# aurelienpierreeng/ansel

Measured on AMD Instinct MI355X. Metric: MPix/s full export pixelpipe (100 MP raw); % MI355X HBM roofline, higher is better.
Workload: dtype f32

## Files before the change

ansel_amd/csrc/diffuse.hip:

```cpp
#include "hip_common.h"

#include <type_traits>
#include "devmath.h"
#include "ieee_inrange.h"
#include "px_colorspaces.h"

#include <math.h>
#include <cstdlib>

namespace ansel
{
int bspline_launch_decompose(int devid, hipStream_t s, const float4 *in, float4 *hf, float4 *lf, int w, int h, int mult,
                             const unsigned *gate = nullptr);
int bspline_launch_decompose3(int devid, hipStream_t s, const void *in, bool in4, float *lf, int w, int h, int mult, unsigned *alpha_flag);
#ifdef ANSEL_HIP_MEASURING
int bspline_launch_decompose2(int devid, hipStream_t s, const float4 *in, float4 *low1, float4 *low2, int w, int h, int mult);
#endif
}
using namespace ansel;

namespace
{

#define DIFFUSE_MAX_SCALES 10
#define BSPLINE_SIGMA 1.0553651328015339f
#define PDE_KAPPA 0.25f

__device__ __forceinline__ float max_first(const float a, const float b) { return a > b ? a : b; }
__device__ __forceinline__ float max_zero(const float v) { return isfinite(v) ? max_first(v, 0.0f) : 0.0f; }
__device__ __forceinline__ int clampi(const int v, const int lo, const int hi) { return v < lo ? lo : (v > hi ? hi : v); }

__device__ __forceinline__ int walk_row(const int b, const int height, const int mult)
{
  if(height <= mult) return b < height ? b : -1;
  const int per_pass = (height + mult - 1) / mult;
  const int row = (b % per_pass) * mult + b / per_pass;
  return row < height ? row : -1;
}

struct pde_args
{
  int width, height, mult;
  float anisotropy[4];
  int kind[4];
  int same02, same13;
  float variance_threshold, regularization;
  float abcd[4], strength;
  int wskip;
  int post_lab;
  float post_m[3][4];
  int approx_div;
  int off;
  const unsigned *gate;
  int gate_sense;
};

#ifdef ANSEL_HIP_MEASURING
#define PDE_APPROX(a) ((a).approx_div != 0)
#define PDE_OFF(a, bit) (((a).off & (bit)) != 0)
#else
#define PDE_APPROX(a) false
#define PDE_OFF(a, bit) false
#endif
__device__ __forceinline__ float div_1ulp(const float x, const float y)
{
  const float r = __builtin_amdgcn_rcpf(y);
  const float q = x * r;
  return __builtin_fmaf(__builtin_fmaf(-y, q, x), r, q);
}

__device__ __forceinline__ float fast_expf(const float x)
{
  const float t = 1065353216.0f + x * 11401300.0f;
  int k = (t > -2147483648.0f && t < 2147483648.0f) ? (int)t : 0;
  k = k > 0 ? k : 0;
  return __int_as_float(k);
}
// ... 56 lines not shown
    w.k1 = a11;
    w.k2 = -w.k0;
    w.k3 = a00;
    w.k4 = -2.0f * (a00 + a11);
  }
  return w;
}

__device__ __forceinline__ float convolve(const kernel5 w, const float p[9])
{
  float d = 0.0f;
  d = w.k0 * p[0] + d;
  d = w.k1 * p[1] + d;
  d = w.k2 * p[2] + d;
  d = w.k3 * p[3] + d;
  d = w.k4 * p[4] + d;
  d = w.k3 * p[5] + d;
  d = w.k2 * p[6] + d;
  d = w.k1 * p[7] + d;
  d = w.k0 * p[8] + d;
  return d;
}

__device__ __forceinline__ float ratio2(const float h, const float l)
{
  const float safe = max_zero(l - 1e-8f) + 1e-8f;
  const float ratio = h / safe;
  return ratio * ratio;
}
__device__ __forceinline__ float4 ratio2_rgb(const float4 h, const float4 l, const float w_ratio, const bool approx = false)
{
  if(approx)
  {
    const float ax = div_1ulp(h.x, max_zero(l.x - 1e-8f) + 1e-8f), ay = div_1ulp(h.y, max_zero(l.y - 1e-8f) + 1e-8f),
                az = div_1ulp(h.z, max_zero(l.z - 1e-8f) + 1e-8f);
    return make_float4(ax * ax, ay * ay, az * az, w_ratio);
  }
  const float sx = max_zero(l.x - 1e-8f) + 1e-8f, sy = max_zero(l.y - 1e-8f) + 1e-8f, sz = max_zero(l.z - 1e-8f) + 1e-8f;
  const float top = __builtin_fmaxf(__builtin_fmaxf(__builtin_fmaxf(__builtin_fabsf(h.x), __builtin_fabsf(h.y)), __builtin_fabsf(h.z)),
                                    __builtin_fmaxf(__builtin_fmaxf(sx, sy), sz));
  float rx, ry, rz;
  if(__builtin_amdgcn_ballot_w64(!(top <= 0x1p64f)) == 0ull)
  {
    rx = ansel_ieee::div_core(h.x, sx);
    ry = ansel_ieee::div_core(h.y, sy);
    rz = ansel_ieee::div_core(h.z, sz);
  }
  else
  {
    rx = h.x / sx;
    ry = h.y / sy;
    rz = h.z / sz;
  }
  return make_float4(rx * rx, ry * ry, rz * rz, w_ratio);
}

#define PDE_MODE_ISOTROPIC (81 + 162)
#define PDE_MODE_DEBLUR (1 + 9 + 81 + 162)
#define PDE_MODE_ISOPHOTE (1 + 3 + 9 + 27 + 81 + 162)
#define PDE_MODE_GRADIENT (2 + 6 + 18 + 54 + 81 + 162)
#define PDE_MODE_WATERCOLOR (9 + 27)
#define PDE_MODE_CONTRAST (2 + 54)
#define PDE_MODE_INPAINT (27)
#define PDE_MODE_FAST (9)
#define PDE_MODES(X) X(PDE_MODE_ISOTROPIC) X(PDE_MODE_DEBLUR) X(PDE_MODE_ISOPHOTE) X(PDE_MODE_GRADIENT) X(PDE_MODE_WATERCOLOR) \
  X(PDE_MODE_CONTRAST) X(PDE_MODE_INPAINT) X(PDE_MODE_FAST)
template <int MODE> struct pde_mode
{
  static __device__ __forceinline__ int kind(const int i, const pde_args &a)
  {
    if constexpr(MODE < 0) return a.kind[i];
    else return (i == 0 ? MODE : (i == 1 ? MODE / 3 : (i == 2 ? MODE / 9 : MODE / 27))) % 3;
  }
  static __device__ __forceinline__ bool same02(const pde_args &a)
  {
    if constexpr(MODE < 0) return a.same02 != 0;
    else return (MODE / 81) % 2 != 0;
  }
  static __device__ __forceinline__ bool same13(const pde_args &a)
  {
    if constexpr(MODE < 0) return a.same13 != 0;
    else return (MODE / 162) % 2 != 0;
  }
};
inline int pde_mode_of(const pde_args &a)
{
  return a.kind[0] + 3 * a.kind[1] + 9 * a.kind[2] + 27 * a.kind[3] + 81 * (a.same02 ? 1 : 0) + 162 * (a.same13 ? 1 : 0);
}

template <int MODE = -1>
__device__ __forceinline__ float pde_channel(const float H[9], const float L[9], float energy, const pde_args &a)
{
  typedef pde_mode<MODE> M;
  energy = max_zero(a.variance_threshold + energy * a.regularization - 1e-8f) + 1e-8f;
  float cos2g = 0.f, sin2g = 0.f, csg = 0.f, cos2l = 0.f, sin2l = 0.f, csl = 0.f, mg = 0.f, ml = 0.f;
  if(M::kind(0, a) | M::kind(2, a)) mg = direction((L[7] - L[1]) * 0.5f, (L[5] - L[3]) * 0.5f, cos2g, sin2g, csg, PDE_APPROX(a));
  if(M::kind(1, a) | M::kind(3, a)) ml = direction((H[7] - H[1]) * 0.5f, (H[5] - H[3]) * 0.5f, cos2l, sin2l, csl, PDE_APPROX(a));
  const kernel5 w0 = order_kernel(M::kind(0, a), fast_expf(-mg * a.anisotropy[0]), csg, cos2g, sin2g);
  const kernel5 w1 = order_kernel(M::kind(1, a), fast_expf(-ml * a.anisotropy[1]), csl, cos2l, sin2l);
  const kernel5 w2 = M::same02(a) ? w0 : order_kernel(M::kind(2, a), fast_expf(-mg * a.anisotropy[2]), csg, cos2g, sin2g);
  const kernel5 w3 = M::same13(a) ? w1 : order_kernel(M::kind(3, a), fast_expf(-ml * a.anisotropy[3]), csl, cos2l, sin2l);
  const float d0 = convolve(w0, L);
  const float d1 = convolve(w1, L);
  const float d2 = convolve(w2, H);
  const float d3 = convolve(w3, H);
  float update = d0 * a.abcd[0];
  update = d1 * a.abcd[1] + update;
  update = d2 * a.abcd[2] + update;
  update = d3 * a.abcd[3] + update;
  const float acc = H[4] * a.strength + (PDE_APPROX(a) ? div_1ulp(update, energy) : update / energy);
  return max_zero(acc + L[4]);
}

__device__ __forceinline__ bool alpha_is_blank(const float4 H4[9], const float4 L4[9])
{
  unsigned bits = 0;
#pragma unroll
  for(int k = 0; k < 9; k++) bits |= __float_as_uint(H4[k].w) | __float_as_uint(L4[k].w);
  return __builtin_amdgcn_ballot_w64(bits != 0) == 0ull;
}

#define PDE_SHARED_MULT 128
template <bool SHARED>
__global__ __launch_bounds__(256) void diffuse_pde(const float4 *__restrict__ hf, const float4 *__restrict__ lf,
                                                   float4 *__restrict__ out, const pde_args a, const int final_pass,
                                                   const unsigned char *__restrict__ mask)
{
  extern __shared__ float4 r2s[];
// ... 140 lines not shown
  if constexpr(H0_4)
    asm volatile("s_waitcnt lgkmcnt(0)\n\ts_nop 4\n\ts_mov_b32 %0, m0\n\t"
                 "s_mov_b32 m0, %6\n\ts_nop 0\n\tglobal_load_lds_dwordx4 %1, %3\n\t"
                 "s_mov_b32 m0, %7\n\ts_nop 0\n\tglobal_load_lds_dwordx3 %2, %4\n\t"
                 "s_mov_b32 m0, %8\n\ts_nop 0\n\tglobal_load_lds_dwordx3 %2, %5\n\t"
                 "s_mov_b32 m0, %0"
                 : "=&s"(keep)
                 : "v"(voff0), "v"(voff), "s"(p0), "s"(p1), "s"(p2), "s"(d0), "s"(d1), "s"(d2)
                 : "memory");
  else
    asm volatile("s_waitcnt lgkmcnt(0)\n\ts_nop 4\n\ts_mov_b32 %0, m0\n\t"
                 "s_mov_b32 m0, %5\n\ts_nop 0\n\tglobal_load_lds_dwordx3 %1, %2\n\t"
                 "s_mov_b32 m0, %6\n\ts_nop 0\n\tglobal_load_lds_dwordx3 %1, %3\n\t"
                 "s_mov_b32 m0, %7\n\ts_nop 0\n\tglobal_load_lds_dwordx3 %1, %4\n\t"
                 "s_mov_b32 m0, %0"
                 : "=&s"(keep)
                 : "v"(voff), "s"(p0), "s"(p1), "s"(p2), "s"(d0), "s"(d1), "s"(d2)
                 : "memory");
}
struct pde_px3
{
  float x, y, z;
};
template <bool HSUB, int MODE, bool DMA, int L3>
__device__ __forceinline__ void pde_strip_body(const float4 *__restrict__ hf, const float4 *__restrict__ hsub,
                                               const float4 *__restrict__ lf, float4 *__restrict__ out, const pde_args &a,
                                               const int final_pass, const unsigned char *__restrict__ mask, const int strip,
                                               const int strips_per_class)
{
  static_assert(L3 == 0 || (HSUB && DMA), "three-float planes: the low-pass chain's LDS-DMA form only");
  if(a.gate && ((*a.gate != 0u) == (a.gate_sense == 1))) return;
  extern __shared__ float4 r2s[];
  pde_px3 *const r2s3 = reinterpret_cast<pde_px3 *>(r2s);
  const int mult = a.mult;
  const int cls = blockIdx.y / strips_per_class, k0s = (blockIdx.y - cls * strips_per_class) * strip;
  const int n_cls = (a.height - cls + mult - 1) / mult;
  if(k0s >= n_cls) return;
  const int nrows = (strip < n_cls - k0s) ? strip : n_cls - k0s;
  const int r_first = cls + k0s * mult;
  const int tx = threadIdx.x, tw = 256 + 2 * mult;
  const int col = (int)blockIdx.x * 256 + tx;
  const bool live = col < a.width;
  const int cols[3] = { clampi(col - mult, 0, a.width - 1), clampi(col, 0, a.width - 1), clampi(col + mult, 0, a.width - 1) };
#define PDE_ROW(v) ((size_t)clampi(r_first + ((v) - 1) * mult, 0, a.height - 1) * a.width)
  float4 Hw[3][3], Lw[3][3];
  constexpr int NPL = HSUB ? 3 : 2;
  const int lane = tx & 63, zw = 64 + 2 * mult;
  float4 *const zone = r2s + PDE_RING * tw + (tx >> 6) * NPL * zw;
  float4 *const zone3 = reinterpret_cast<float4 *>(reinterpret_cast<char *>(r2s) + (size_t)PDE_RING * tw * 12) + (tx >> 6) * 3 * zw;
  using lds_f4_ptr = __attribute__((address_space(3))) float4 *;
  const unsigned zone_lds = !DMA ? 0u : (unsigned)__builtin_amdgcn_readfirstlane((int)(unsigned)(__UINTPTR_TYPE__)(lds_f4_ptr)(
                                           L3 ? zone3 : zone));
  const unsigned off_main = (unsigned)cols[0] * 16u, off_halo = (unsigned)clampi(col - mult + 64, 0, a.width - 1) * 16u;
  auto dma_row = [&](const int v) {
// ... 9 lines not shown
        pde_dma_planes3<L3 == 2>(b0, b1, b2, L3 == 2 ? off_halo : h3, h3, zone_lds + 1024u, zone_lds + p0 + 1024u, zone_lds + p1 + 1024u);
      return;
    }
    const unsigned pl = (unsigned)zw * 16u;
    pde_dma_planes<NPL>(hf + y, hsub + y, lf + y, off_main, zone_lds, zone_lds + pl, zone_lds + (NPL - 1) * pl);
    if(lane < 2 * mult)
      pde_dma_planes<NPL>(hf + y, hsub + y, lf + y, off_halo, zone_lds + 1024u, zone_lds + pl + 1024u, zone_lds + (NPL - 1) * pl + 1024u);
  };
  struct
  {
    float4 o;
    size_t idx;
    bool have;
  } pending;
  pending.have = false;
  auto store = [&](const size_t i, const float4 o) {
    if(final_pass) nt_store(out + i, o);
    else if constexpr(L3 != 0)
    {
      float *const p3 = (float *)out + 3 * i;
      p3[0] = o.x;
      p3[1] = o.y;
      p3[2] = o.z;
    }
    else out[i] = o;
  };
  auto fetch_row = [&](const int v, auto slot_tag) {
    constexpr int SL = decltype(slot_tag)::value;
    const size_t y = PDE_ROW(v);
    float4 c[3], low[3];
    if constexpr(DMA)
    {
      asm volatile("s_waitcnt vmcnt(0)" : : : "memory");
      if constexpr(L3 != 0)
      {
#pragma unroll
        for(int jj = 0; jj < 3; jj++)
        {
          const int x = lane + jj * mult;
          const float4 v0 = zone3[x], v1 = zone3[zw + x], v2 = zone3[2 * zw + x];
          c[jj] = make_float4(v0.x, v0.y, v0.z, 0.0f);
          low[jj] = make_float4(v1.x, v1.y, v1.z, 0.0f);
          Lw[SL][jj] = make_float4(v2.x, v2.y, v2.z, 0.0f);
        }
      }
      else
// ... 18 lines not shown
    {
#pragma unroll
      for(int jj = 0; jj < 3; jj++)
      {
        c[jj] = hf[y + cols[jj]];
        if(HSUB) low[jj] = hsub[y + cols[jj]];
        Lw[SL][jj] = lf[y + cols[jj]];
      }
    }
    __builtin_amdgcn_sched_barrier(0);
#pragma unroll
    for(int jj = 0; jj < 3; jj++)
      Hw[SL][jj] = HSUB ? make_float4(c[jj].x - low[jj].x, c[jj].y - low[jj].y, c[jj].z - low[jj].z, c[jj].w - low[jj].w) : c[jj];
    float4 *const ring = r2s + (v % PDE_RING) * tw;
    auto ratios = [&](const float4 h, const float4 l) {
      const bool blank = a.wskip && __builtin_amdgcn_ballot_w64((__float_as_uint(h.w) | __float_as_uint(l.w)) != 0) == 0ull;
      return ratio2_rgb(h, l, blank ? 0.0f : ratio2(h.w, l.w), PDE_APPROX(a));
    };
    if(PDE_OFF(a, 4)) return;
    if constexpr(L3 != 0)
    {
      pde_px3 *const ring3 = r2s3 + (v % PDE_RING) * tw;
      auto put = [&](const int x, const float4 h, const float4 l) {
        const float4 r = ratio2_rgb(h, l, 0.0f, PDE_APPROX(a));
        ring3[x] = { r.x, r.y, r.z };
      };
      put(tx + mult, Hw[SL][1], Lw[SL][1]);
      if(tx < mult) put(tx, Hw[SL][0], Lw[SL][0]);
      if(tx >= 256 - mult) put(tx + 2 * mult, Hw[SL][2], Lw[SL][2]);
      return;
    }
    ring[tx + mult] = ratios(Hw[SL][1], Lw[SL][1]);
    if(tx < mult) ring[tx] = ratios(Hw[SL][0], Lw[SL][0]);
    if(tx >= 256 - mult) ring[tx + 2 * mult] = ratios(Hw[SL][2], Lw[SL][2]);
  };
  auto row_step = [&](auto t_tag, const int kk) {
    constexpr int T = decltype(t_tag)::value, S0 = T, S1 = (T + 1) % 3, S2 = (T + 2) % 3;
    constexpr bool WIDE_READS = MODE >= 0 && !(((MODE % 3) | ((MODE / 9) % 3)) && (((MODE / 3) % 3) | ((MODE / 27) % 3)));
    fetch_row(kk + 2, std::integral_constant<int, S2>());
    if constexpr(DMA)
    {
      if(pending.have)
      {
        store(pending.idx, pending.o);
        pending.have = false;
      }
      if(kk + 1 < nrows) dma_row(kk + 3);
// ... 38 lines not shown
      {
        const float4 r = ring[jj * mult];
        energy.x += r.x;
        energy.y += r.y;
        energy.z += r.z;
        if(!(blank && a.wskip)) energy.w += r.w;
      }
      if(!WIDE_READS || ii >= 1) asm volatile("" : "+v"(energy.x), "+v"(energy.y), "+v"(energy.z), "+v"(energy.w) : : "memory");
    }
    const size_t idx = (size_t)row * a.width + col;
    float4 o;
    if(L3 == 0 && mask && !mask[idx])
    {
      const float4 h = H4[4], l = L4[4];
      o = make_float4(max_zero(h.x + l.x), max_zero(h.y + l.y), max_zero(h.z + l.z), max_zero(h.w + l.w));
    }
    else if(PDE_OFF(a, 16))
      o = make_float4(H4[4].x + energy.x, L4[4].y + energy.y, H4[0].z + energy.z, L4[8].w);
    else
    {
      float H[9], L[9];
#pragma unroll
      for(int k = 0; k < 9; k++) { H[k] = H4[k].x; L[k] = L4[k].x; }
      o.x = pde_channel<MODE>(H, L, energy.x, a);
#pragma unroll
      for(int k = 0; k < 9; k++) { H[k] = H4[k].y; L[k] = L4[k].y; }
      o.y = pde_channel<MODE>(H, L, energy.y, a);
#pragma unroll
      for(int k = 0; k < 9; k++) { H[k] = H4[k].z; L[k] = L4[k].z; }
      o.z = pde_channel<MODE>(H, L, energy.z, a);
      if(blank)
        o.w = 0.0f;
      else
      {
#pragma unroll
        for(int k = 0; k < 9; k++) { H[k] = H4[k].w; L[k] = L4[k].w; }
        o.w = pde_channel<MODE>(H, L, energy.w, a);
      }
    }
    if(a.post_lab) o = px_rgb_to_lab(o, a.post_m);
    pending.o = o;
    pending.idx = idx;
    pending.have = true;
  };
  if constexpr(DMA) dma_row(0);
  fetch_row(0, std::integral_constant<int, 0>());
  if constexpr(DMA) dma_row(1);
  fetch_row(1, std::integral_constant<int, 1>());
  if constexpr(DMA) dma_row(2);
  for(int kk = 0; kk < nrows; kk += 3)
  {
    row_step(std::integral_constant<int, 0>(), kk);
    if(kk + 1 < nrows) row_step(std::integral_constant<int, 1>(), kk + 1);
    if(kk + 2 < nrows) row_step(std::integral_constant<int, 2>(), kk + 2);
  }
  if constexpr(DMA) asm volatile("s_waitcnt vmcnt(0)" : : : "memory");
  if(pending.have) store(pending.idx, pending.o);
#undef PDE_ROW
}

template <bool HSUB, int MODE, bool DMA = false>
__global__ __launch_bounds__(256, 3) void diffuse_pde_strip(const float4 *__restrict__ hf, const float4 *__restrict__ hsub,
                                                         const float4 *__restrict__ lf,
                                                         float4 *__restrict__ out, const pde_args a, const int final_pass,
                                                         const unsigned char *__restrict__ mask, const int strip,
                                                         const int strips_per_class)
{
  pde_strip_body<HSUB, MODE, DMA, 0>(hf, hsub, lf, out, a, final_pass, mask, strip, strips_per_class);
}
template <int MODE, bool H0_4>
__global__ __launch_bounds__(256, 3) void diffuse_pde_strip3(const float4 *__restrict__ hf, const float4 *__restrict__ hsub,
                                                          const float4 *__restrict__ lf, float4 *__restrict__ out, const pde_args a,
                                                          const int final_pass, const int strip, const int strips_per_class)
{
  pde_strip_body<true, MODE, true, H0_4 ? 2 : 1>(hf, hsub, lf, out, a, final_pass, nullptr, strip, strips_per_class);
}

__device__ __forceinline__ uint32_t splitmix32(const uint64_t seed)
{
  uint64_t result = (seed ^ (seed >> 33)) * 0x62a9d9ed799705f5ull;
  result = (result ^ (result >> 28)) * 0xcb24d0a5c88c35b3ull;
  return (uint32_t)(result >> 32);
}

__device__ __forceinline__ float xoshiro128plus(uint32_t state[4])
{
  const uint32_t result = state[0] + state[3];
  const uint32_t t = state[1] << 9;
  state[2] ^= state[0];
  state[3] ^= state[1];
  state[1] ^= state[2];
  state[0] ^= state[3];
  state[2] ^= t;
  state[3] = (state[3] << 11) | (state[3] >> 21);
  return (float)(result >> 8) * 0x1.0p-24f;
}

__device__ __forceinline__ float gaussian_noise(const float mu, const float sigma, const bool flip, uint32_t state[4])
// ... 73 lines not shown
int diffuse_halo_rows(const dt_hip_piece_t *piece, const dt_hip_diffuse_data_t *d)
{
  if(!(d->iscale > 0.0f) || !(piece->roi_in.scale > 0.0)) return -1;
  const int scales = scales_of(piece, d);
  const int it_req = (int)ceilf((float)d->iterations);
  const int iterations = it_req > 1 ? it_req : 1;
  return iterations * 3 * ((1 << scales) - 1);
}
}

extern "C" {

int dt_hip_iop_diffuse_process(int devid, const dt_hip_piece_t *piece, const dt_hip_diffuse_data_t *d,
                               dt_hip_mem_t dev_in, dt_hip_mem_t dev_out)
{
  return diffuse_process_rows(devid, piece, d, 0, dev_in, dev_out);
}

}

namespace ansel
{
static void *g_diffuse_probe = nullptr;

static int diffuse_run(int devid, const dt_hip_piece_t *piece, const dt_hip_diffuse_data_t *d, int first_row, dt_hip_mem_t dev_in,
                       dt_hip_mem_t dev_out, const dt_hip_lab_data_t *post_lab);
int diffuse_process_rows(int devid, const dt_hip_piece_t *piece, const dt_hip_diffuse_data_t *d, int first_row,
                         dt_hip_mem_t dev_in, dt_hip_mem_t dev_out)
{
  return diffuse_run(devid, piece, d, first_row, dev_in, dev_out, nullptr);
}
int diffuse_process_post_lab(int devid, const dt_hip_piece_t *piece, const dt_hip_diffuse_data_t *d, dt_hip_mem_t dev_in,
                             dt_hip_mem_t dev_out, const dt_hip_lab_data_t *lab)
{
  if(!lab || measuring_env("ANSEL_HIP_PDE_PER_ROW")) return DT_HIP_INVALID_ARG;
  return diffuse_run(devid, piece, d, 0, dev_in, dev_out, lab);
}
static int diffuse_run(int devid, const dt_hip_piece_t *piece, const dt_hip_diffuse_data_t *d, int first_row, dt_hip_mem_t dev_in,
                       dt_hip_mem_t dev_out, const dt_hip_lab_data_t *post_lab)
{
  if(!valid_device(devid) || !piece || !d || !dev_in || !dev_out) return DT_HIP_INVALID_ARG;
  if(piece->channels != 4)
  {
    set_last_error("diffuse: needs a 4-channel float input");
    return DT_HIP_INVALID_ARG;
  }
// ... 29 lines not shown
    const char *const approx_env = measuring_env("ANSEL_HIP_PDE_APPROX_DIV");
    a.approx_div = approx_env && atoi(approx_env) != 0;
    const char *const off_env = measuring_env("ANSEL_HIP_PDE_OFF");
    a.off = off_env ? atoi(off_env) : 0;
  }
  const float user_aniso[4] = { d->anisotropy_first, d->anisotropy_second, d->anisotropy_third, d->anisotropy_fourth };
  for(int k = 0; k < 4; k++)
  {
    a.anisotropy[k] = sqf(user_aniso[k]);
    a.kind[k] = user_aniso[k] == 0.0f ? 0 : (user_aniso[k] > 0.0f ? 1 : 2);
  }
  a.same02 = a.kind[0] == a.kind[2] && a.anisotropy[0] == a.anisotropy[2];
  a.same13 = a.kind[1] == a.kind[3] && a.anisotropy[1] == a.anisotropy[3];
  const float regularization = powf(10.0f, d->regularization) - 1.0f;
  a.variance_threshold = powf(10.0f, d->variance_threshold);
  const float speed[4] = { d->first, d->second, d->third, d->fourth };

  hipStream_t st = stream_of(devid);
  const float4 *src = (const float4 *)dev_in;
  const int mode0 = pde_mode_of(a);
  const bool three = err == DT_HIP_SUCCESS && lf_chain && !no_dma && !(d->threshold > 0.0f) && (1 << (scales - 1)) <= PDE_DMA_MAX_MULT &&
                     !(iterations == 1 && dev_in == dev_out) && !measuring_env("ANSEL_HIP_PDE_GENERIC") &&
                     (mode0 == PDE_MODE_DEBLUR || mode0 == PDE_MODE_ISOTROPIC);
  unsigned *alpha_flag = nullptr;
  if(three)
  {
    alpha_flag = (unsigned *)dt_hip_alloc_device_buffer(devid, sizeof(unsigned));
    if(!alpha_flag) err = DT_HIP_SYSMEM_ALLOCATION;
    else if(hipMemsetAsync(alpha_flag, 0, sizeof(unsigned), st) != hipSuccess) err = DT_HIP_DEFAULT_ERROR;
  }
  unsigned char *mask = nullptr;
  float4 *inpainted = nullptr;
  if(err == DT_HIP_SUCCESS && d->threshold > 0.0f)
  {
    const size_t np = (size_t)w * h;
    mask = (unsigned char *)dt_hip_alloc_device_buffer(devid, np);
    inpainted = tmp[1] ? tmp[1] : (tmp[1] = (float4 *)dt_hip_alloc_device_buffer(devid, plane));
    if(!mask || !inpainted) err = DT_HIP_SYSMEM_ALLOCATION;
    else
    {
      launch_scope ls(devid, "diffuse_inpaint");
      diffuse_inpaint<<<pixel_grid(np), 256, 0, st>>>(src, inpainted, mask, d->threshold, np, (size_t)w, (size_t)first_row * w);
      err = check_launch("diffuse_inpaint");
      src = inpainted;
    }
  }
  for(int seq = three ? 0 : 1; seq < 2 && err == DT_HIP_SUCCESS; seq++)
  {
  const bool p3 = seq == 0;
  a.gate = alpha_flag;
  a.gate_sense = p3 ? 1 : 2;
  if(three) src = (const float4 *)dev_in;
// ... 5 lines not shown
    const bool chain = lf_chain && (const float4 *)dst != src;
    if(!chain && !lf[1])
    {
      lf[1] = (float4 *)dt_hip_alloc_device_buffer(devid, plane);
      if(!lf[1])
      {
        err = DT_HIP_SYSMEM_ALLOCATION;
        break;
      }
    }
    for(int s = 0; s < scales && err == DT_HIP_SUCCESS; s++)
    {
#ifdef ANSEL_HIP_MEASURING
      static const bool pairs = measuring_env("ANSEL_HIP_BSPLINE_PAIRS") != nullptr;
      if(chain && pairs && s + 1 < scales && (s == 0 || s == 2))
      {
        err = bspline_launch_decompose2(devid, st, level, hf[s], hf[s + 1], w, h, 1 << s);
        s++;
        level = residual = hf[s];
        continue;
      }
#endif
      float4 *low = chain ? hf[s] : lf[s % 2];
      if(p3) err = bspline_launch_decompose3(devid, st, level, it == 0 && s == 0, (float *)low, w, h, 1 << s, alpha_flag);
      else err = bspline_launch_decompose(devid, st, level, chain ? nullptr : hf[s], low, w, h, 1 << s, alpha_flag);
      level = low;
      residual = low;
    }
    float4 *pp[2] = { residual == lf[1] ? lf[0] : lf[1], residual };
    const float4 *cur = residual;
    int count = 0;
    for(int s = scales - 1; s >= 0 && err == DT_HIP_SUCCESS; s--, count++)
    {
      const float real_radius = sigma_at_step(BSPLINE_SIGMA, (unsigned)s) * zoom;
      a.regularization = regularization / 9.0f * sqf(real_radius);
      const float norm = expf(-sqf(real_radius - (float)d->radius_center) / sqf((float)d->radius));
      for(int k = 0; k < 4; k++) a.abcd[k] = speed[k] * PDE_KAPPA * norm;
      a.strength = d->sharpness * norm + 1.0f;
      a.mult = 1 << s;
      a.post_lab = 0;
      if(post_lab && s == 0 && it == iterations - 1)
      {
        a.post_lab = 1;
        memcpy(a.post_m, post_lab->matrix, sizeof(a.post_m));
      }
      float4 *to = (s == 0) ? dst : (chain ? (count % 2 == 0 ? lf[0] : hf[s + 1]) : pp[count % 2]);
      const int rows = (h <= a.mult) ? h : ((h + a.mult - 1) / a.mult) * a.mult;
// ... 11 lines not shown
          if(strip_env) strip = atoi(strip_env);
#endif
          while(strip > 4 && (size_t)gx * classes * ((per_class + strip - 1) / strip) < 2048) strip /= 2;
          const int spc = (per_class + strip - 1) / strip;
          size_t ring = (size_t)PDE_RING * (256 + 2 * a.mult) * sizeof(float4);
#ifdef ANSEL_HIP_MEASURING
          static const char *const pad_env = measuring_env("ANSEL_HIP_PDE_LDS_PAD");
          if(pad_env) ring += (size_t)atoi(pad_env);
#endif
          static const bool generic = measuring_env("ANSEL_HIP_PDE_GENERIC") != nullptr;
          const int mode = generic ? -1 : pde_mode_of(a);
          const dim3 sgrid(gx, classes * spc);
          const float4 *const h0 = chain ? (s == 0 ? src : hf[s - 1]) : hf[s], *const h1 = chain ? hf[s] : nullptr;
#define PDE_LAUNCH(HS, MD) diffuse_pde_strip<HS, MD><<<sgrid, 256, ring, st>>>(h0, h1, cur, to, a, s == 0, mask, strip, spc)
          const bool dma = chain && a.mult <= PDE_DMA_MAX_MULT && !no_dma;
          const size_t ring_dma = ring + (size_t)4 * 3 * (64 + 2 * a.mult) * sizeof(float4);
#define PDE_LAUNCH_DMA(MD) diffuse_pde_strip<true, MD, true><<<sgrid, 256, ring_dma, st>>>(h0, h1, cur, to, a, s == 0, mask, strip, spc)
          bool launched = false;
          if(p3)
          {
            const bool h0_4 = it == 0 && s == 0;
            const size_t lds3 = (size_t)PDE_RING * (256 + 2 * a.mult) * 12 + (size_t)4 * 3 * (64 + 2 * a.mult) * 16;
            const int last = s == 0 && it == iterations - 1;
#define PDE_LAUNCH3(MD, H4) diffuse_pde_strip3<MD, H4><<<sgrid, 256, lds3, st>>>(h0, h1, cur, to, a, last, strip, spc)
            if(mode == PDE_MODE_DEBLUR)
            {
              if(h0_4) PDE_LAUNCH3(PDE_MODE_DEBLUR, true);
              else PDE_LAUNCH3(PDE_MODE_DEBLUR, false);
            }
            else
            {
              if(h0_4) PDE_LAUNCH3(PDE_MODE_ISOTROPIC, true);
              else PDE_LAUNCH3(PDE_MODE_ISOTROPIC, false);
            }
#undef PDE_LAUNCH3
            launched = true;
          }
#define PDE_CASE(MD)                     \
  if(!launched && mode == (MD))          \
  {                                      \
    if(dma) PDE_LAUNCH_DMA(MD);          \
    else if(chain) PDE_LAUNCH(true, MD); \
    else PDE_LAUNCH(false, MD);          \
    launched = true;                     \
  }
          PDE_MODES(PDE_CASE)
#undef PDE_CASE
// ... 5 lines not shown
          }
#undef PDE_LAUNCH_DMA
#undef PDE_LAUNCH
        }
        else if(a.mult <= PDE_SHARED_MULT)
          diffuse_pde<true><<<grid, 256, (size_t)3 * (256 + 2 * a.mult) * sizeof(float4), st>>>(hf[s], cur, to, a, s == 0, mask);
        else
          diffuse_pde<false><<<grid, 256, 0, st>>>(hf[s], cur, to, a, s == 0, mask);
      }
      err = check_launch("diffuse_pde");
      cur = to;
    }
    src = dst;
  }
  }
  for(int s = 0; s < scales; s++)
    if(hf[s]) dt_hip_release_mem_object(hf[s]);
  for(int k = 0; k < 2; k++)
  {
    if(lf[k]) dt_hip_release_mem_object(lf[k]);
    if(tmp[k]) dt_hip_release_mem_object(tmp[k]);
  }
  if(mask) dt_hip_release_mem_object(mask);
  if(alpha_flag)
  {
    if(g_diffuse_probe && err == DT_HIP_SUCCESS && hipMemcpyAsync(g_diffuse_probe, alpha_flag, sizeof(unsigned), hipMemcpyDeviceToDevice, st) != hipSuccess)
      err = DT_HIP_DEFAULT_ERROR;
    dt_hip_release_mem_object(alpha_flag);
  }
  else if(g_diffuse_probe && err == DT_HIP_SUCCESS && hipMemsetAsync(g_diffuse_probe, 0xff, sizeof(unsigned), st) != hipSuccess)
    err = DT_HIP_DEFAULT_ERROR;
  return err;
}

}

extern "C" {

int dt_hip_test_diffuse_probe(void *sink)
{
  ansel::g_diffuse_probe = sink;
  return DT_HIP_SUCCESS;
}

void dt_hip_iop_diffuse_tiling(const dt_hip_piece_t *piece, const dt_hip_diffuse_data_t *d, dt_hip_tiling_t *tiling)
{
  const int scales = scales_of(piece, d);
  tiling->factor = 6.0625f + scales;
  tiling->factor_cl = 6.0625f + scales;
  tiling->maxbuf = 1.0f;
  tiling->maxbuf_cl = 1.0f;
  tiling->overhead = 0;
  tiling->overlap = 1 << scales;
  tiling->xalign = 1;
  tiling->yalign = 1;
}

}
```

ansel_amd/csrc/diffuse_bspline.hip:

```cpp
#include "hip_common.h"

#include <cstdlib>

using namespace ansel;

namespace
{

__device__ __forceinline__ float max_first(const float a, const float b) { return a > b ? a : b; }
__device__ __forceinline__ int clampi(const int v, const int lo, const int hi) { return v < lo ? lo : (v > hi ? hi : v); }

__device__ __forceinline__ float tap5(const float a, const float b, const float c, const float d, const float e)
{
  const float s = 0.0625f * a + 0.25f * b + 0.375f * c + 0.25f * d + 0.0625f * e;
  return max_first(0.0f, s);
}
__device__ __forceinline__ float4 tap5(const float4 a, const float4 b, const float4 c, const float4 d, const float4 e)
{
  return make_float4(tap5(a.x, b.x, c.x, d.x, e.x), tap5(a.y, b.y, c.y, d.y, e.y), tap5(a.z, b.z, c.z, d.z, e.z),
                     tap5(a.w, b.w, c.w, d.w, e.w));
}

__device__ __forceinline__ int walk_row(const int b, const int height, const int mult)
{
// ... 152 lines not shown
    c = d;
    d = e;
    e = n1;
    a2 = b2;
    b2 = c2;
    c2 = d2;
    d2 = e2;
    e2 = n2;
  }
#undef BS_ROW
}

struct bs_px3
{
  float x, y, z;
};
__device__ __forceinline__ bs_px3 tap5(const bs_px3 a, const bs_px3 b, const bs_px3 c, const bs_px3 d, const bs_px3 e)
{
  return { tap5(a.x, b.x, c.x, d.x, e.x), tap5(a.y, b.y, c.y, d.y, e.y), tap5(a.z, b.z, c.z, d.z, e.z) };
}
template <int R, int T, bool IN4>
__global__ __launch_bounds__(256) void bspline_decompose_strip3(const void *__restrict__ in_v, bs_px3 *__restrict__ lf,
                                                                const int width, const int height, const int strip,
                                                                const int strips_per_class, unsigned *__restrict__ alpha_flag)
{
  static_assert(R * T == 256, "a workgroup's columns: one span of 256");
  constexpr int mult = R;
  if(!IN4 && *alpha_flag != 0u) return;
  __shared__ bs_px3 vert[2][(T + 4) * R + 2];
  const float4 *const in4 = static_cast<const float4 *>(in_v);
  const bs_px3 *const in3 = static_cast<const bs_px3 *>(in_v);
  unsigned alpha_bits = 0;
  auto at = [&](const size_t i) -> bs_px3 {
    if constexpr(IN4)
    {
      const float4 v = in4[i];
      alpha_bits |= __float_as_uint(v.w);
      return { v.x, v.y, v.z };
    }
    else
      return in3[i];
  };
  const int cls = blockIdx.y / strips_per_class, k0s = (blockIdx.y - cls * strips_per_class) * strip;
  const int n_cls = (height - cls + mult - 1) / mult;
  if(k0s >= n_cls) return;
  const int nrows = (strip < n_cls - k0s) ? strip : n_cls - k0s;
  const int r_first = cls + k0s * mult;
  const int k0 = (int)blockIdx.x * T;
  const int tid = threadIdx.x;
  const int r = tid % R, k = tid / R;
  const int col = r + (k0 + k) * mult;
  const bool own = col < width;
  int col2 = -1, slot2 = 0;
  if(tid < 4 * R)
  {
    const int hr = tid % R, hs = tid / R;
    const int hk = hs < 2 ? hs - 2 : T + hs - 2;
    const int hcol = hr + (k0 + hk) * mult;
    if(hcol >= 0 && hcol < width)
    {
// ... 31 lines not shown
    d2 = at(BS_ROW(1) + col2);
    e2 = at(BS_ROW(2) + col2);
  }
  for(int kk = 0; kk < nrows; kk++)
  {
    const int row = r_first + kk * mult;
    const bool more = kk + 1 < nrows;
    bs_px3 n1 = z, n2 = z;
    if(more && own) n1 = at(BS_ROW(kk + 3) + col);
    if(more && second) n2 = at(BS_ROW(kk + 3) + col2);
    bs_px3 *const V = vert[kk & 1];
    if(own) V[(k + 2) * R + r] = tap5(a, b, c, d, e);
    if(second) V[slot2] = tap5(a2, b2, c2, d2, e2);
    __syncthreads();
    if(own)
    {
      bs_px3 t[5];
#pragma unroll
      for(int s = -2; s <= 2; s++)
      {
        const int cc = col + s * mult;
        t[s + 2] = cc < 0 ? V[(T + 4) * R] : (cc > width - 1 ? V[(T + 4) * R + 1] : V[(k + s + 2) * R + r]);
      }
      lf[(size_t)row * width + col] = tap5(t[0], t[1], t[2], t[3], t[4]);
    }
    a = b;
    b = c;
    c = d;
    d = e;
    e = n1;
    a2 = b2;
    b2 = c2;
    c2 = d2;
    d2 = e2;
    e2 = n2;
  }
#undef BS_ROW
  if(IN4 && __builtin_amdgcn_ballot_w64(alpha_bits != 0u) != 0ull && (tid & 63) == 0) atomicOr(alpha_flag, 1u);
}

#ifdef ANSEL_HIP_MEASURING
__device__ __forceinline__ float4 bs_row_taps(const float4 *__restrict__ V, const int col, const int step, const int origin,
                                              const int width)
{
  float4 t[5];
#pragma unroll
  for(int j = 0; j < 5; j++) t[j] = V[clampi(col + (j - 2) * step, 0, width - 1) - origin];
  return tap5(t[0], t[1], t[2], t[3], t[4]);
}

template <int M, int AHEAD>
__global__ __launch_bounds__(320) void bspline_decompose2_strip(const float4 *__restrict__ in, float4 *__restrict__ low1,
                                                                float4 *__restrict__ low2, const int width, const int height,
                                                                const int strip, const int strips_per_class)
{
  constexpr int M2 = 2 * M, WA = 256 + 12 * M, WB = 256 + 8 * M;
  static_assert(WA <= 320, "a lane a column");
  __shared__ float4 VA[2][WA], VC[2][WB];
  const int c0 = (int)blockIdx.x * 256;
  const int cls = blockIdx.y / strips_per_class, k0s = (blockIdx.y - cls * strips_per_class) * strip;
  const int n_cls = (height - cls + M2 - 1) / M2;
// ... 112 lines not shown
  static const char *const ahead_env = measuring_env("ANSEL_HIP_BSPLINE_AHEAD");
  const int ahead = ahead_env ? atoi(ahead_env) : 1;
#define BS_PAIR(MM) \
  switch(ahead) \
  { \
    case 2: bspline_decompose2_strip<MM, 2><<<grid, 320, 0, s>>>(in, low1, low2, w, h, strip, spc); break; \
    case 4: bspline_decompose2_strip<MM, 4><<<grid, 320, 0, s>>>(in, low1, low2, w, h, strip, spc); break; \
    case 3: bspline_decompose2_strip<MM, 3><<<grid, 320, 0, s>>>(in, low1, low2, w, h, strip, spc); break; \
    default: bspline_decompose2_strip<MM, 1><<<grid, 320, 0, s>>>(in, low1, low2, w, h, strip, spc); break; \
  }
  if(mult == 1)
  {
    BS_PAIR(1);
  }
  else
  {
    BS_PAIR(4);
  }
#undef BS_PAIR
  return check_launch("diffuse_decompose");
}
#endif

int bspline_launch_decompose3(int devid, hipStream_t s, const void *in, bool in4, float *lf, int w, int h, int mult, unsigned *alpha_flag)
{
  (void)devid;
  if(mult != 1 && mult != 2 && mult != 4 && mult != 8 && mult != 16) return DT_HIP_INVALID_ARG;
  if(in4 && mult != 1) return DT_HIP_INVALID_ARG;
  const int classes = h < mult ? h : mult, per_class = (h + mult - 1) / mult;
  const int gx = (w + 255) / 256;
  int strip = 32;
  while(strip > 4 && (size_t)gx * classes * ((per_class + strip - 1) / strip) < 2048) strip /= 2;
  const int spc = (per_class + strip - 1) / strip;
  const dim3 grid(gx, classes * spc);
  launch_scope ls(devid, "diffuse_decompose");
  bs_px3 *const out = reinterpret_cast<bs_px3 *>(lf);
  if(in4) bspline_decompose_strip3<1, 256, true><<<grid, 256, 0, s>>>(in, out, w, h, strip, spc, alpha_flag);
  else if(mult == 1) bspline_decompose_strip3<1, 256, false><<<grid, 256, 0, s>>>(in, out, w, h, strip, spc, alpha_flag);
  else if(mult == 2) bspline_decompose_strip3<2, 128, false><<<grid, 256, 0, s>>>(in, out, w, h, strip, spc, alpha_flag);
  else if(mult == 4) bspline_decompose_strip3<4, 64, false><<<grid, 256, 0, s>>>(in, out, w, h, strip, spc, alpha_flag);
  else if(mult == 8) bspline_decompose_strip3<8, 32, false><<<grid, 256, 0, s>>>(in, out, w, h, strip, spc, alpha_flag);
  else bspline_decompose_strip3<16, 16, false><<<grid, 256, 0, s>>>(in, out, w, h, strip, spc, alpha_flag);
  return check_launch("diffuse_decompose");
}

int bspline_launch_decompose(int devid, hipStream_t s, const float4 *in, float4 *hf, float4 *lf, int w, int h, int mult,
                             const unsigned *gate)
{
  const int steps = (w + mult - 1) / mult;
  launch_scope ls(devid, "diffuse_decompose");
#ifdef ANSEL_HIP_MEASURING
  static const bool per_row = getenv("ANSEL_HIP_BSPLINE_PER_ROW") != nullptr;
  if(per_row)
  {
    const int rows = (h <= mult) ? h : ((h + mult - 1) / mult) * mult;
    if(mult == 1)
      bspline_decompose<1, 256><<<dim3(xcd_pad((steps + 255) / 256), rows), 256, 0, s>>>(in, hf, lf, w, h, mult, 1, (steps + 255) / 256);
    else if(mult == 2)
      bspline_decompose<2, 128><<<dim3(xcd_pad((steps + 127) / 128), rows), 256, 0, s>>>(in, hf, lf, w, h, mult, 1, (steps + 127) / 128);
    else if(mult == 4)
      bspline_decompose<4, 64><<<dim3(xcd_pad((steps + 63) / 64), rows), 256, 0, s>>>(in, hf, lf, w, h, mult, 1, (steps + 63) / 64);
    else
    {
      const int groups = mult / 8;
      bspline_decompose<8, 32><<<dim3(xcd_pad(((steps + 31) / 32) * groups), rows), 256, 0, s>>>(in, hf, lf, w, h, mult, groups,
// ... 19 lines not shown
```

ansel_amd/csrc/ieee_inrange.h:

```cpp
#pragma once

namespace ansel_ieee
{

__device__ __forceinline__ float div_core(const float a, const float b)
{
  float r = __builtin_amdgcn_rcpf(b);
  const float e = __builtin_fmaf(-b, r, 1.0f);
  r = __builtin_fmaf(e, r, r);
  float q = a * r;
  const float e2 = __builtin_fmaf(-b, q, a);
  q = __builtin_fmaf(e2, r, q);
  const float e3 = __builtin_fmaf(-b, q, a);
  return __builtin_fmaf(e3, r, q);
}

__device__ __forceinline__ float rcp_core(const float b)
{
  float r = __builtin_amdgcn_rcpf(b);
  const float e = __builtin_fmaf(-b, r, 1.0f);
  r = __builtin_fmaf(e, r, r);
  const float e2 = __builtin_fmaf(-b, r, 1.0f);
  const float q = __builtin_fmaf(e2, r, r);
  const float e3 = __builtin_fmaf(-b, q, 1.0f);
// ... 10 lines not shown
  const float q = n * y1;
  const float q1 = __builtin_fmaf(__builtin_fmaf(-d, q, n), y1, q);
  const float q2 = __builtin_fmaf(__builtin_fmaf(-d, q1, n), y1, q1);
  return __builtin_amdgcn_div_fixupf(q2, d, n);
}

__device__ __forceinline__ float sqrt_core(const float x)
{
  const float s = __builtin_amdgcn_sqrtf(x);
  const float down = __uint_as_float(__float_as_uint(s) - 1u), up = __uint_as_float(__float_as_uint(s) + 1u);
  const float r_down = __builtin_fmaf(-down, s, x);
  float t = (0.0f >= r_down) ? down : s;
  const float r_up = __builtin_fmaf(-up, s, x);
  t = (0.0f < r_up) ? up : t;
  return t;
}

__device__ __forceinline__ bool zero_or_above_2m96(const float x)
{
  const unsigned u = __float_as_uint(x);
  return u == 0u || (u - 0x0f800000u) <= (0x7f7fffffu - 0x0f800000u);
}

}
```

Measured before the change: 1625.

## Add range-gated fused PDE kernel with simplified ratio division and isotropic Laplacian

Introduces a fused variant of the three-float PDE strip kernel that uses a fixed isotropic Laplacian stencil and an unconditional refined division for the ratio term. Its correctness rests on a value-range premise. The B-spline decomposition and the fused kernel both check for out-of-range values and set a device flag. Both the fused and the original kernel are launched each time, gated on that flag so only one does real work. This trims the per-pixel ALU cost of the PDE step in exchange for range checks, an extra launch that exits early, and an atomic flag.

```diff
diff --git a/ansel_amd/csrc/diffuse.hip b/ansel_amd/csrc/diffuse.hip
--- a/ansel_amd/csrc/diffuse.hip
+++ b/ansel_amd/csrc/diffuse.hip
@@ -12,7 +12,8 @@
 {
 int bspline_launch_decompose(int devid, hipStream_t s, const float4 *in, float4 *hf, float4 *lf, int w, int h, int mult,
                              const unsigned *gate = nullptr);
-int bspline_launch_decompose3(int devid, hipStream_t s, const void *in, bool in4, float *lf, int w, int h, int mult, unsigned *alpha_flag);
+int bspline_launch_decompose3(int devid, hipStream_t s, const void *in, bool in4, float *lf, int w, int h, int mult, unsigned *alpha_flag,
+                              unsigned *range_flag);
 #ifdef ANSEL_HIP_MEASURING
 int bspline_launch_decompose2(int devid, hipStream_t s, const float4 *in, float4 *low1, float4 *low2, int w, int h, int mult);
 #endif
@@ -53,6 +54,8 @@
   int off;
   const unsigned *gate;
   int gate_sense;
+  unsigned *range;
+  int range_sense;
 };
 
 #ifdef ANSEL_HIP_MEASURING
@@ -155,6 +158,20 @@
   return d;
 }
 
+__device__ __forceinline__ float convolve_iso_fused(const float p[9])
+{
+  float d = __builtin_fmaf(0.25f, p[0], 0.0f);
+  d = __builtin_fmaf(0.5f, p[1], d);
+  d = __builtin_fmaf(0.25f, p[2], d);
+  d = __builtin_fmaf(0.5f, p[3], d);
+  d = -3.0f * p[4] + d;
+  d = __builtin_fmaf(0.5f, p[5], d);
+  d = __builtin_fmaf(0.25f, p[6], d);
+  d = __builtin_fmaf(0.5f, p[7], d);
+  d = __builtin_fmaf(0.25f, p[8], d);
+  return d;
+}
+
 __device__ __forceinline__ float ratio2(const float h, const float l)
 {
   const float safe = max_zero(l - 1e-8f) + 1e-8f;
@@ -186,6 +203,16 @@
     rz = h.z / sz;
   }
   return make_float4(rx * rx, ry * ry, rz * rz, w_ratio);
+}
+
+#ifndef ANSEL_PDE_FUSED_KEEPS_RATIO_TEST
+#define ANSEL_PDE_FUSED_KEEPS_RATIO_TEST 0
+#endif
+__device__ __forceinline__ float4 ratio2_rgb_r(const float4 h, const float4 l)
+{
+  const float sx = max_first(l.x - 1e-8f, 0.0f) + 1e-8f, sy = max_first(l.y - 1e-8f, 0.0f) + 1e-8f, sz = max_first(l.z - 1e-8f, 0.0f) + 1e-8f;
+  const float rx = ansel_ieee::div_core(h.x, sx), ry = ansel_ieee::div_core(h.y, sy), rz = ansel_ieee::div_core(h.z, sz);
+  return make_float4(rx * rx, ry * ry, rz * rz, 0.0f);
 }
 
 #define PDE_MODE_ISOTROPIC (81 + 162)
@@ -221,7 +248,7 @@
   return a.kind[0] + 3 * a.kind[1] + 9 * a.kind[2] + 27 * a.kind[3] + 81 * (a.same02 ? 1 : 0) + 162 * (a.same13 ? 1 : 0);
 }
 
-template <int MODE = -1>
+template <int MODE = -1, bool FUSED = false>
 __device__ __forceinline__ float pde_channel(const float H[9], const float L[9], float energy, const pde_args &a)
 {
   typedef pde_mode<MODE> M;
@@ -233,10 +260,14 @@
   const kernel5 w1 = order_kernel(M::kind(1, a), fast_expf(-ml * a.anisotropy[1]), csl, cos2l, sin2l);
   const kernel5 w2 = M::same02(a) ? w0 : order_kernel(M::kind(2, a), fast_expf(-mg * a.anisotropy[2]), csg, cos2g, sin2g);
   const kernel5 w3 = M::same13(a) ? w1 : order_kernel(M::kind(3, a), fast_expf(-ml * a.anisotropy[3]), csl, cos2l, sin2l);
-  const float d0 = convolve(w0, L);
-  const float d1 = convolve(w1, L);
-  const float d2 = convolve(w2, H);
-  const float d3 = convolve(w3, H);
+  static_assert(!FUSED || MODE >= 0, "the fused Laplacians: kinds spelled at compile time only");
+  constexpr bool F0 = FUSED && (MODE % 3) == 0, F1 = FUSED && ((MODE / 3) % 3) == 0;
+  constexpr bool F2 = (FUSED && (MODE / 81) % 2) ? F0 : (FUSED && ((MODE / 9) % 3) == 0);
+  constexpr bool F3 = (FUSED && (MODE / 162) % 2) ? F1 : (FUSED && ((MODE / 27) % 3) == 0);
+  const float d0 = F0 ? convolve_iso_fused(L) : convolve(w0, L);
+  const float d1 = F1 ? convolve_iso_fused(L) : convolve(w1, L);
+  const float d2 = F2 ? convolve_iso_fused(H) : convolve(w2, H);
+  const float d3 = F3 ? convolve_iso_fused(H) : convolve(w3, H);
   float update = d0 * a.abcd[0];
   update = d1 * a.abcd[1] + update;
   update = d2 * a.abcd[2] + update;
@@ -423,14 +454,17 @@
 {
   float x, y, z;
 };
-template <bool HSUB, int MODE, bool DMA, int L3>
+template <bool HSUB, int MODE, bool DMA, int L3, bool FUSED = false>
 __device__ __forceinline__ void pde_strip_body(const float4 *__restrict__ hf, const float4 *__restrict__ hsub,
                                                const float4 *__restrict__ lf, float4 *__restrict__ out, const pde_args &a,
                                                const int final_pass, const unsigned char *__restrict__ mask, const int strip,
                                                const int strips_per_class)
 {
   static_assert(L3 == 0 || (HSUB && DMA), "three-float planes: the low-pass chain's LDS-DMA form only");
+  static_assert(!FUSED || L3 != 0, "premise R is established for the three-float planes only");
   if(a.gate && ((*a.gate != 0u) == (a.gate_sense == 1))) return;
+  if(L3 != 0 && a.range && ((*a.range != 0u) == (a.range_sense == 1))) return;
+  unsigned long long outside = 0ull;
   extern __shared__ float4 r2s[];
   pde_px3 *const r2s3 = reinterpret_cast<pde_px3 *>(r2s);
   const int mult = a.mult;
@@ -486,6 +520,7 @@
       p3[0] = o.x;
       p3[1] = o.y;
       p3[2] = o.z;
+      if constexpr(FUSED) outside |= __builtin_amdgcn_ballot_w64(ansel_ieee::outside_r3<true>(o.x, o.y, o.z));
     }
     else out[i] = o;
   };
@@ -550,7 +585,7 @@
     {
       pde_px3 *const ring3 = r2s3 + (v % PDE_RING) * tw;
       auto put = [&](const int x, const float4 h, const float4 l) {
-        const float4 r = ratio2_rgb(h, l, 0.0f, PDE_APPROX(a));
+        const float4 r = (FUSED && !ANSEL_PDE_FUSED_KEEPS_RATIO_TEST) ? ratio2_rgb_r(h, l) : ratio2_rgb(h, l, 0.0f, PDE_APPROX(a));
         ring3[x] = { r.x, r.y, r.z };
       };
       put(tx + mult, Hw[SL][1], Lw[SL][1]);
@@ -635,20 +670,20 @@
       float H[9], L[9];
 #pragma unroll
       for(int k = 0; k < 9; k++) { H[k] = H4[k].x; L[k] = L4[k].x; }
-      o.x = pde_channel<MODE>(H, L, energy.x, a);
+      o.x = pde_channel<MODE, FUSED>(H, L, energy.x, a);
 #pragma unroll
       for(int k = 0; k < 9; k++) { H[k] = H4[k].y; L[k] = L4[k].y; }
-      o.y = pde_channel<MODE>(H, L, energy.y, a);
+      o.y = pde_channel<MODE, FUSED>(H, L, energy.y, a);
 #pragma unroll
       for(int k = 0; k < 9; k++) { H[k] = H4[k].z; L[k] = L4[k].z; }
-      o.z = pde_channel<MODE>(H, L, energy.z, a);
+      o.z = pde_channel<MODE, FUSED>(H, L, energy.z, a);
       if(blank)
         o.w = 0.0f;
       else
       {
 #pragma unroll
         for(int k = 0; k < 9; k++) { H[k] = H4[k].w; L[k] = L4[k].w; }
-        o.w = pde_channel<MODE>(H, L, energy.w, a);
+        o.w = pde_channel<MODE, FUSED>(H, L, energy.w, a);
       }
     }
     if(a.post_lab) o = px_rgb_to_lab(o, a.post_m);
@@ -669,6 +704,8 @@
   }
   if constexpr(DMA) asm volatile("s_waitcnt vmcnt(0)" : : : "memory");
   if(pending.have) store(pending.idx, pending.o);
+  if constexpr(FUSED)
+    if(outside != 0ull && lane == 0) atomicOr(a.range, 1u);
 #undef PDE_ROW
 }
 
@@ -687,6 +724,13 @@
                                                           const int final_pass, const int strip, const int strips_per_class)
 {
   pde_strip_body<true, MODE, true, H0_4 ? 2 : 1>(hf, hsub, lf, out, a, final_pass, nullptr, strip, strips_per_class);
+}
+template <int MODE, bool H0_4>
+__global__ __launch_bounds__(256, 3) void diffuse_pde_fused3(const float4 *__restrict__ hf, const float4 *__restrict__ hsub,
+                                                          const float4 *__restrict__ lf, float4 *__restrict__ out, const pde_args a,
+                                                          const int final_pass, const int strip, const int strips_per_class)
+{
+  pde_strip_body<true, MODE, true, H0_4 ? 2 : 1, true>(hf, hsub, lf, out, a, final_pass, nullptr, strip, strips_per_class);
 }
 
 __device__ __forceinline__ uint32_t splitmix32(const uint64_t seed)
@@ -806,6 +850,7 @@
 namespace ansel
 {
 static void *g_diffuse_probe = nullptr;
+static void *g_diffuse_range_probe = nullptr;
 
 static int diffuse_run(int devid, const dt_hip_piece_t *piece, const dt_hip_diffuse_data_t *d, int first_row, dt_hip_mem_t dev_in,
                        dt_hip_mem_t dev_out, const dt_hip_lab_data_t *post_lab);
@@ -881,12 +926,14 @@
   const bool three = err == DT_HIP_SUCCESS && lf_chain && !no_dma && !(d->threshold > 0.0f) && (1 << (scales - 1)) <= PDE_DMA_MAX_MULT &&
                      !(iterations == 1 && dev_in == dev_out) && !measuring_env("ANSEL_HIP_PDE_GENERIC") &&
                      (mode0 == PDE_MODE_DEBLUR || mode0 == PDE_MODE_ISOTROPIC);
-  unsigned *alpha_flag = nullptr;
+  unsigned *alpha_flag = nullptr, *range_flag = nullptr;
   if(three)
   {
     alpha_flag = (unsigned *)dt_hip_alloc_device_buffer(devid, sizeof(unsigned));
-    if(!alpha_flag) err = DT_HIP_SYSMEM_ALLOCATION;
-    else if(hipMemsetAsync(alpha_flag, 0, sizeof(unsigned), st) != hipSuccess) err = DT_HIP_DEFAULT_ERROR;
+    range_flag = (unsigned *)dt_hip_alloc_device_buffer(devid, sizeof(unsigned));
+    if(!alpha_flag || !range_flag) err = DT_HIP_SYSMEM_ALLOCATION;
+    else if(hipMemsetAsync(alpha_flag, 0, sizeof(unsigned), st) != hipSuccess || hipMemsetAsync(range_flag, 0, sizeof(unsigned), st) != hipSuccess)
+      err = DT_HIP_DEFAULT_ERROR;
   }
   unsigned char *mask = nullptr;
   float4 *inpainted = nullptr;
@@ -938,7 +985,7 @@
       }
 #endif
       float4 *low = chain ? hf[s] : lf[s % 2];
-      if(p3) err = bspline_launch_decompose3(devid, st, level, it == 0 && s == 0, (float *)low, w, h, 1 << s, alpha_flag);
+      if(p3) err = bspline_launch_decompose3(devid, st, level, it == 0 && s == 0, (float *)low, w, h, 1 << s, alpha_flag, range_flag);
       else err = bspline_launch_decompose(devid, st, level, chain ? nullptr : hf[s], low, w, h, 1 << s, alpha_flag);
       level = low;
       residual = low;
@@ -996,7 +1043,16 @@
             const bool h0_4 = it == 0 && s == 0;
             const size_t lds3 = (size_t)PDE_RING * (256 + 2 * a.mult) * 12 + (size_t)4 * 3 * (64 + 2 * a.mult) * 16;
             const int last = s == 0 && it == iterations - 1;
-#define PDE_LAUNCH3(MD, H4) diffuse_pde_strip3<MD, H4><<<sgrid, 256, lds3, st>>>(h0, h1, cur, to, a, last, strip, spc)
+#define PDE_LAUNCH3(MD, H4)                                                                      \
+  do                                                                                             \
+  {                                                                                              \
+    a.range = range_flag;                                                                        \
+    a.range_sense = 1;                                                                           \
+    diffuse_pde_fused3<MD, H4><<<sgrid, 256, lds3, st>>>(h0, h1, cur, to, a, last, strip, spc);  \
+    a.range_sense = 2;                                                                           \
+    diffuse_pde_strip3<MD, H4><<<sgrid, 256, lds3, st>>>(h0, h1, cur, to, a, last, strip, spc);  \
+    a.range = nullptr;                                                                           \
+  } while(0)
             if(mode == PDE_MODE_DEBLUR)
             {
               if(h0_4) PDE_LAUNCH3(PDE_MODE_DEBLUR, true);
@@ -1048,6 +1104,15 @@
     if(tmp[k]) dt_hip_release_mem_object(tmp[k]);
   }
   if(mask) dt_hip_release_mem_object(mask);
+  if(range_flag)
+  {
+    if(g_diffuse_range_probe && err == DT_HIP_SUCCESS
+       && hipMemcpyAsync(g_diffuse_range_probe, range_flag, sizeof(unsigned), hipMemcpyDeviceToDevice, st) != hipSuccess)
+      err = DT_HIP_DEFAULT_ERROR;
+    dt_hip_release_mem_object(range_flag);
+  }
+  else if(g_diffuse_range_probe && err == DT_HIP_SUCCESS && hipMemsetAsync(g_diffuse_range_probe, 0xff, sizeof(unsigned), st) != hipSuccess)
+    err = DT_HIP_DEFAULT_ERROR;
   if(alpha_flag)
   {
     if(g_diffuse_probe && err == DT_HIP_SUCCESS && hipMemcpyAsync(g_diffuse_probe, alpha_flag, sizeof(unsigned), hipMemcpyDeviceToDevice, st) != hipSuccess)
@@ -1067,6 +1132,18 @@
 {
   ansel::g_diffuse_probe = sink;
   return DT_HIP_SUCCESS;
+}
+
+int dt_hip_test_diffuse_range_probe(void *sink)
+{
+  ansel::g_diffuse_range_probe = sink;
+  return DT_HIP_SUCCESS;
+}
+
+int dt_hip_test_diffuse_rows(int devid, const dt_hip_piece_t *piece, const dt_hip_diffuse_data_t *d, int first_row, dt_hip_mem_t dev_in,
+                             dt_hip_mem_t dev_out)
+{
+  return ansel::diffuse_process_rows(devid, piece, d, first_row, dev_in, dev_out);
 }
 
 void dt_hip_iop_diffuse_tiling(const dt_hip_piece_t *piece, const dt_hip_diffuse_data_t *d, dt_hip_tiling_t *tiling)
diff --git a/ansel_amd/csrc/diffuse_bspline.hip b/ansel_amd/csrc/diffuse_bspline.hip
--- a/ansel_amd/csrc/diffuse_bspline.hip
+++ b/ansel_amd/csrc/diffuse_bspline.hip
@@ -1,4 +1,5 @@
 #include "hip_common.h"
+#include "ieee_inrange.h"
 
 #include <cstdlib>
 
@@ -198,7 +199,8 @@
 template <int R, int T, bool IN4>
 __global__ __launch_bounds__(256) void bspline_decompose_strip3(const void *__restrict__ in_v, bs_px3 *__restrict__ lf,
                                                                 const int width, const int height, const int strip,
-                                                                const int strips_per_class, unsigned *__restrict__ alpha_flag)
+                                                                const int strips_per_class, unsigned *__restrict__ alpha_flag,
+                                                                unsigned *__restrict__ range_flag)
 {
   static_assert(R * T == 256, "a workgroup's columns: one span of 256");
   constexpr int mult = R;
@@ -207,11 +209,13 @@
   const float4 *const in4 = static_cast<const float4 *>(in_v);
   const bs_px3 *const in3 = static_cast<const bs_px3 *>(in_v);
   unsigned alpha_bits = 0;
+  bool outside = false;
   auto at = [&](const size_t i) -> bs_px3 {
     if constexpr(IN4)
     {
       const float4 v = in4[i];
       alpha_bits |= __float_as_uint(v.w);
+      outside |= ansel_ieee::outside_r3(v.x, v.y, v.z);
       return { v.x, v.y, v.z };
     }
     else
@@ -289,7 +293,9 @@
         const int cc = col + s * mult;
         t[s + 2] = cc < 0 ? V[(T + 4) * R] : (cc > width - 1 ? V[(T + 4) * R + 1] : V[(k + s + 2) * R + r]);
       }
-      lf[(size_t)row * width + col] = tap5(t[0], t[1], t[2], t[3], t[4]);
+      const bs_px3 o = tap5(t[0], t[1], t[2], t[3], t[4]);
+      lf[(size_t)row * width + col] = o;
+      outside |= ansel_ieee::outside_r3(o.x, o.y, o.z);
     }
     a = b;
     b = c;
@@ -304,6 +310,7 @@
   }
 #undef BS_ROW
   if(IN4 && __builtin_amdgcn_ballot_w64(alpha_bits != 0u) != 0ull && (tid & 63) == 0) atomicOr(alpha_flag, 1u);
+  if(__builtin_amdgcn_ballot_w64(outside) != 0ull && (tid & 63) == 0) atomicOr(range_flag, 1u);
 }
 
 #ifdef ANSEL_HIP_MEASURING
@@ -462,7 +469,8 @@
 }
 #endif
 
-int bspline_launch_decompose3(int devid, hipStream_t s, const void *in, bool in4, float *lf, int w, int h, int mult, unsigned *alpha_flag)
+int bspline_launch_decompose3(int devid, hipStream_t s, const void *in, bool in4, float *lf, int w, int h, int mult, unsigned *alpha_flag,
+                              unsigned *range_flag)
 {
   (void)devid;
   if(mult != 1 && mult != 2 && mult != 4 && mult != 8 && mult != 16) return DT_HIP_INVALID_ARG;
@@ -475,12 +483,12 @@
   const dim3 grid(gx, classes * spc);
   launch_scope ls(devid, "diffuse_decompose");
   bs_px3 *const out = reinterpret_cast<bs_px3 *>(lf);
-  if(in4) bspline_decompose_strip3<1, 256, true><<<grid, 256, 0, s>>>(in, out, w, h, strip, spc, alpha_flag);
-  else if(mult == 1) bspline_decompose_strip3<1, 256, false><<<grid, 256, 0, s>>>(in, out, w, h, strip, spc, alpha_flag);
-  else if(mult == 2) bspline_decompose_strip3<2, 128, false><<<grid, 256, 0, s>>>(in, out, w, h, strip, spc, alpha_flag);
-  else if(mult == 4) bspline_decompose_strip3<4, 64, false><<<grid, 256, 0, s>>>(in, out, w, h, strip, spc, alpha_flag);
-  else if(mult == 8) bspline_decompose_strip3<8, 32, false><<<grid, 256, 0, s>>>(in, out, w, h, strip, spc, alpha_flag);
-  else bspline_decompose_strip3<16, 16, false><<<grid, 256, 0, s>>>(in, out, w, h, strip, spc, alpha_flag);
+  if(in4) bspline_decompose_strip3<1, 256, true><<<grid, 256, 0, s>>>(in, out, w, h, strip, spc, alpha_flag, range_flag);
+  else if(mult == 1) bspline_decompose_strip3<1, 256, false><<<grid, 256, 0, s>>>(in, out, w, h, strip, spc, alpha_flag, range_flag);
+  else if(mult == 2) bspline_decompose_strip3<2, 128, false><<<grid, 256, 0, s>>>(in, out, w, h, strip, spc, alpha_flag, range_flag);
+  else if(mult == 4) bspline_decompose_strip3<4, 64, false><<<grid, 256, 0, s>>>(in, out, w, h, strip, spc, alpha_flag, range_flag);
+  else if(mult == 8) bspline_decompose_strip3<8, 32, false><<<grid, 256, 0, s>>>(in, out, w, h, strip, spc, alpha_flag, range_flag);
+  else bspline_decompose_strip3<16, 16, false><<<grid, 256, 0, s>>>(in, out, w, h, strip, spc, alpha_flag, range_flag);
   return check_launch("diffuse_decompose");
 }
 
diff --git a/ansel_amd/csrc/ieee_inrange.h b/ansel_amd/csrc/ieee_inrange.h
--- a/ansel_amd/csrc/ieee_inrange.h
+++ b/ansel_amd/csrc/ieee_inrange.h
@@ -56,4 +56,12 @@
   return u == 0u || (u - 0x0f800000u) <= (0x7f7fffffu - 0x0f800000u);
 }
 
+template <bool NONNEG = false> __device__ __forceinline__ bool outside_r3(const float x, const float y, const float z)
+{
+  const unsigned keep = NONNEG ? 0xffffffffu : 0x7fffffffu;
+  const unsigned mx = __float_as_uint(x) & keep, my = __float_as_uint(y) & keep, mz = __float_as_uint(z) & keep;
+  const unsigned lo = min(min(mx - 1u, my - 1u), mz - 1u), hi = max(max(mx, my), mz);
+  return lo < 0x0d800000u - 1u || hi > 0x5f000000u;
 }
+
+}
```

Measured after the change: 1638 (median of 6 runs). About the same (+0.8%).
